# zdebruine/RcppML

Measured on AMD Instinct MI355X. Metric: ALS updates/sec (cols solved/s), k=64 sparse NMF, higher is better.
Workload: dtype f32; 1 GPU; configs[1]: simulateNMF 20000x100000 (x1 GPUs, column shards) 1%-dense CSC, k=64, MSE, coordinate-descent NNLS (cd_maxit=100, cd_tol=1e-8), L1 row normalisation, loss every iteration; rows=20000, cols_per_gpu=100000, nnz_per_gpu=20054852, k=64, solver=cd, cd_variant=auto, parallelism=column-shard x1

## Files before the change

### include/rcppml_gpu.h

```cpp
#ifndef RCPPML_GPU_H
#define RCPPML_GPU_H

#include <stddef.h>
#include <stdint.h>

#ifdef __cplusplus
extern "C" {
#endif

#define RCPPML_GPU_API __attribute__((visibility("default")))


RCPPML_GPU_API void rcppml_gpu_detect(int* num_gpus, double* total_mem_mb, double* free_mem_mb,
                                      int* max_gpus, int* out_status);

#define RCPPML_NMF_UNIFIED_ARGS                                                                    \
    const int* col_ptr, const int* row_idx, const double* values, int* m, int* n, int* nnz, int* k, \
        double* W, double* H, double* d, int* max_iter, double* tol, double* L1_H, double* L1_W,   \
        double* L2_H, double* L2_W, double* L21_H, double* L21_W, double* ortho_H, double* ortho_W, \
        double* ub_H, double* ub_W, int* cd_maxit, int* verbose, int* seed, int* loss_every,       \
        int* patience, int* nonneg_W, int* nonneg_H, int* loss_type, double* huber_delta,          \
        int* irls_max_iter, double* irls_tol, int* norm_type, int* projective, int* symmetric,     \
        int* solver_mode, const int* graph_W_p, const int* graph_W_i, const double* graph_W_x,     \
        int* graph_W_dim, int* graph_W_nnz, double* graph_W_lambda, const int* graph_H_p,          \
// ... 186 lines not shown
RCPPML_GPU_API void rcppml_gpu_consensus_double(const double* W_stack, int* m, int* k, int* reps, int* method, int* knn,
        double* out_consensus, int* out_labels, int* out_status);
RCPPML_GPU_API void rcppml_gpu_hclust_average_double(const double* dist, int* m, int* k_cut, int* out_merge, double* out_height,
        int* out_clusters, double* out_cophenetic, int* out_status);

RCPPML_GPU_API void rcppml_gpu_compute_target_double(const double* H, const int* labels, int* k, int* n, int* n_classes, int* whiten,
        double* out_target, double* out_shift, int* out_counts, int* out_status);
RCPPML_GPU_API void rcppml_gpu_refine_correct_double(const double* H, const int* labels, int* k, int* n, int* n_classes, int* whiten,
        double* lambda, int* nonneg, double* out_H_corr, double* out_target, int* out_status);
RCPPML_GPU_API void rcppml_gpu_refine_wfit_double(const int* col_ptr, const int* row_idx, const double* values, int* nnz,
        const double* dense, int* m, int* n, int* k, const double* d, const double* H_corr, int* nonneg, double* out_W,
        int* out_status);
RCPPML_GPU_API void rcppml_gpu_refine_double(const int* col_ptr, const int* row_idx, const double* values, int* nnz,
        const double* dense, int* m, int* n, int* k, const double* W_T, const double* d, const double* H, const int* labels,
        int* n_classes, double* lambda, int* cycles, int* nonneg, int* whiten, double* out_W, double* out_d, double* out_H,
        double* out_H_corr, int* out_status);

RCPPML_GPU_API void rcppml_gpu_nmf_zi_double(const int* col_ptr, const int* row_idx, const double* values, int* m, int* n, int* nnz,
        int* k, double* W, double* H, double* d, int* max_iter, double* tol, double* L1_H, double* L1_W, double* L2_H, double* L2_W,
        double* ub_H, double* ub_W, int* cd_maxit, double* cd_tol, int* verbose, int* patience, int* nonneg_W, int* nonneg_H,
        int* loss_type, int* irls_max_iter, double* irls_tol, int* norm_type, int* dispersion_mode, double* gp_theta_init,
        double* gp_theta_max, double* gp_theta_min, double* nb_size_init, double* nb_size_max, double* nb_size_min, int* sort_model,
        int* zi_mode, int* zi_em_iters, double* loss_history, double* out_theta, int* out_theta_len, double* out_pi, int* out_pi_len,
        int* out_iter, int* out_converged, double* out_loss, double* out_tol, int* out_status);
RCPPML_GPU_API void rcppml_gpu_zi_em_double(const int* col_ptr, const int* row_idx, const double* values, int* nnz, int* m, int* n,
        int* k, const double* W_T, const double* d, const double* H, double* disp, int* loss_type, int* zi_mode, int* zi_em_iters,
        double* theta_min, double* pi, double* out_imputed, int* out_status);

RCPPML_GPU_API const char* rcppml_gpu_last_error(void);

typedef struct rcppml_hip_ctx rcppml_hip_ctx;

enum { RCPPML_F32 = 0, RCPPML_F64 = 1 };
enum { RCPPML_CD_AUTO = 0 ,
       RCPPML_CD_LANE = 1 ,
       RCPPML_CD_WAVE = 2 ,
       RCPPML_CD_GROUP = 5 ,
       RCPPML_CD_MFMA16 = 7 ,
       RCPPML_CD_MFMA = 6 ,
       RCPPML_CD_LMF = 8  };

RCPPML_GPU_API int rcppml_hip_ctx_create(rcppml_hip_ctx** out, int device, void* stream);
RCPPML_GPU_API void rcppml_hip_ctx_destroy(rcppml_hip_ctx* ctx);
RCPPML_GPU_API int rcppml_hip_ctx_sync(rcppml_hip_ctx* ctx);
RCPPML_GPU_API int rcppml_hip_ctx_stats(rcppml_hip_ctx* ctx, int reset, unsigned long long* out4);
RCPPML_GPU_API int rcppml_hip_ctx_irls_stats(rcppml_hip_ctx* ctx, int reset, unsigned long long* out2);
RCPPML_GPU_API int rcppml_hip_ctx_irls_sweep_stats(rcppml_hip_ctx* ctx, int reset, unsigned long long* out1);
RCPPML_GPU_API int rcppml_hip_ctx_cd_step_stats(rcppml_hip_ctx* ctx, int reset, unsigned long long* out2);
enum { RCPPML_OPT_CD_COUNT_NOOP = 1 ,
       RCPPML_OPT_CD_LMF_LANE_GROUPS = 2 ,
       RCPPML_OPT_CD_LMF_WAVES_PER_SIMD = 3 ,
       RCPPML_OPT_CD_NO_LMF = 4 ,
       RCPPML_OPT_IRLS_COLUMNS_PER_WAVE = 5,
       RCPPML_OPT_SMALL_GIVE_UP = 6  };
RCPPML_GPU_API int rcppml_hip_ctx_set_option(rcppml_hip_ctx* ctx, int option, int value);

RCPPML_GPU_API int rcppml_hip_transpose_csc(rcppml_hip_ctx* ctx, int dtype, int rows, int cols, const int* col_ptr,
                                            const int* row_idx, const void* values, int* t_col_ptr, int* t_row_idx,
                                            void* t_values);
RCPPML_GPU_API int rcppml_hip_transpose_csc_sort(rcppml_hip_ctx* ctx, int rows, int cols, int64_t nnz, const int* col_ptr,
                                                 const int* row_idx, int* t_col_ptr, int* sorted_pos);
RCPPML_GPU_API int rcppml_hip_transpose_csc_gather(rcppml_hip_ctx* ctx, int dtype, int cols, int64_t nnz, const int* col_ptr,
                                                   const int* sorted_pos, const void* values, int* t_row_idx, void* t_values);
RCPPML_GPU_API int rcppml_hip_cast(rcppml_hip_ctx* ctx, int dtype_src, const void* src, int dtype_dst, void* dst, int64_t n);

RCPPML_GPU_API int rcppml_hip_gram(rcppml_hip_ctx* ctx, int dtype, const void* F, int k, int64_t r,
                                   double eps, double l2, void* G);

RCPPML_GPU_API int rcppml_hip_rhs(rcppml_hip_ctx* ctx, int dtype, const int* col_ptr,
                                  const int* row_idx, const void* values, int64_t ncols,
                                  const void* F, int k, void* B);

typedef struct rcppml_rhs_plan rcppml_rhs_plan;
RCPPML_GPU_API int rcppml_hip_rhs_plan_create(rcppml_hip_ctx* ctx, int dtype, const int* col_ptr, const int* row_idx,
                                              const void* values, int64_t ncols, int64_t nrows, int k, int partitions,
                                              int slots, rcppml_rhs_plan** out_plan);
RCPPML_GPU_API int rcppml_hip_rhs_plan_kind(const rcppml_rhs_plan* plan);
RCPPML_GPU_API int rcppml_hip_rhs_plan_create_indices(rcppml_hip_ctx* ctx, int dtype, const int* col_ptr, const int* row_idx, int64_t ncols,
                                                      int64_t nrows, int k, int partitions, int slots, rcppml_rhs_plan** out_plan);
RCPPML_GPU_API int rcppml_hip_rhs_plan_set_values(rcppml_hip_ctx* ctx, rcppml_rhs_plan* plan, const void* values);
RCPPML_GPU_API void rcppml_hip_rhs_plan_destroy(rcppml_rhs_plan* plan);
RCPPML_GPU_API int rcppml_hip_rhs_plan_info(const rcppml_rhs_plan* plan, double* out11);
RCPPML_GPU_API int rcppml_hip_rhs_planned(rcppml_hip_ctx* ctx, const rcppml_rhs_plan* plan, const void* F, void* B);

RCPPML_GPU_API int rcppml_hip_solve_cd(rcppml_hip_ctx* ctx, int dtype, const void* G, const void* B,
                                       void* X, int k, int64_t ncols, double l1_pre, int warm,
                                       int zero_init, double l1_cd, double l2_cd, int nonneg,
                                       int maxit, double tol, double ub_cd, double ub_post,
                                       int variant, int* sweeps_out, const int* col_order);

RCPPML_GPU_API int rcppml_hip_order_columns(rcppml_hip_ctx* ctx, const int* sweeps, int64_t ncols, int* order);

RCPPML_GPU_API int rcppml_hip_solve_chol(rcppml_hip_ctx* ctx, int dtype, const void* G,
                                         const void* B, void* X, int k, int64_t ncols,
                                         double l1_pre, int nonneg, double ub_post);

RCPPML_GPU_API int rcppml_hip_row_norms(rcppml_hip_ctx* ctx, int dtype, const void* X, int k,
                                        int64_t ncols, int norm_type, void* out);
RCPPML_GPU_API int rcppml_hip_apply_scaling(rcppml_hip_ctx* ctx, int dtype, void* X, int k,
                                            int64_t ncols, int norm_type, const void* sums, void* d);

RCPPML_GPU_API int rcppml_hip_scale_order(rcppml_hip_ctx* ctx, int dtype, void* X, int k, int64_t ncols, int norm_type,
                                          void* sums, void* d, const int* sweeps, int* order);

RCPPML_GPU_API int rcppml_hip_sumsq(rcppml_hip_ctx* ctx, int dtype, const void* x, int64_t len,
                                    double* out);

// ... 119 lines not shown
```

### rcppml_amd/_abi.py

```python
import ctypes as C
import os

import numpy as np

_HERE = os.path.dirname(os.path.abspath(__file__))
LIB_PATH = os.environ.get("RCPPML_GPU_LIB_PATH") or os.path.join(_HERE, "lib", "RcppML_gpu.so")
_lib = None

F32, F64 = 0, 1
CD_AUTO, CD_LANE, CD_WAVE, CD_GROUP, CD_MFMA, CD_MFMA16, CD_LMF = 0, 1, 2, 5, 6, 7, 8
OPT_CD_COUNT_NOOP, OPT_CD_LMF_LANE_GROUPS, OPT_CD_LMF_WAVES_PER_SIMD, OPT_CD_NO_LMF, OPT_IRLS_COLUMNS_PER_WAVE, OPT_SMALL_GIVE_UP = 1, 2, 3, 4, 5, 6

EXPORTED_SYMBOLS = [
    "rcppml_gpu_detect", "rcppml_gpu_nmf_unified_float", "rcppml_gpu_nmf_unified_double", "rcppml_gpu_nmf_ex",
    "rcppml_gpu_nmf_cv_unified_float", "rcppml_gpu_nmf_cv_unified_double", "rcppml_gpu_nmf_cv_ex", "rcppml_gpu_nmf_cv_irls_ex", "rcppml_gpu_nmf_cv_masked_ex", "rcppml_hip_ctx_set_cv_mask", "rcppml_gpu_nmf_zerocopy_double",
    "rcppml_gpu_nnls_double", "rcppml_gpu_evaluate_mse_double", "rcppml_gpu_nmf_profile_double", "rcppml_gpu_last_error",
    "rcppml_hip_ctx_create", "rcppml_hip_ctx_destroy", "rcppml_hip_ctx_sync", "rcppml_hip_ctx_stats", "rcppml_hip_ctx_irls_stats", "rcppml_hip_ctx_irls_sweep_stats", "rcppml_hip_ctx_cd_step_stats", "rcppml_hip_ctx_set_option", "rcppml_hip_transpose_csc", "rcppml_hip_transpose_csc_sort", "rcppml_hip_transpose_csc_gather", "rcppml_hip_cast", "rcppml_hip_gram", "rcppml_hip_rhs",
    "rcppml_hip_solve_cd", "rcppml_hip_order_columns", "rcppml_hip_solve_chol", "rcppml_hip_row_norms", "rcppml_hip_apply_scaling",
    "rcppml_hip_sumsq", "rcppml_hip_loss_mse", "rcppml_hip_solve_masked", "rcppml_hip_loss_nonzeros", "rcppml_hip_loss_masked",
    "rcppml_hip_solve_irls_nb", "rcppml_hip_nb_size_update", "rcppml_hip_nb_size_update_loss", "rcppml_hip_nb_loss", "rcppml_hip_solve_irls", "rcppml_hip_rhs_plan_kind", "rcppml_hip_irls_loss", "rcppml_hip_apply_l21", "rcppml_hip_angular_posthoc", "rcppml_hip_solve_cv", "rcppml_hip_cv_test_error", "rcppml_hip_solve_cv_irls", "rcppml_hip_cv_irls_loss", "rcppml_hip_cv_gp_theta_update", "rcppml_hip_mul_rows", "rcppml_hip_apply_graph_reg", "rcppml_hip_dispersion_update", "rcppml_hip_vec_global", "rcppml_hip_spz_info", "rcppml_hip_spz_decode",
    "rcppml_sp_read_gpu", "rcppml_sp_free_gpu", "rcppml_hip_rhs_dense", "rcppml_gpu_nmf_dense_unified_float",
    "rcppml_gpu_nmf_dense_unified_double",
    "rcppml_hip_rhs_plan_create", "rcppml_hip_rhs_plan_create_indices", "rcppml_hip_rhs_plan_set_values", "rcppml_hip_rhs_plan_destroy", "rcppml_hip_rhs_plan_info", "rcppml_hip_rhs_planned",
    "rcppml_gpu_nmf_target", "rcppml_hip_axpy", "rcppml_hip_add_diag", "rcppml_hip_clip_upper",
    "rcppml_hip_scale_order", "rcppml_hip_gram_loss_mse", "rcppml_hip_tail_scale_gram", "rcppml_hip_tail_scale_gram_loss",
    "rcppml_hip_als_small_eligible", "rcppml_hip_als_small_fit",
    "rcppml_gpu_bipartition_double", "rcppml_gpu_dclust_double", "rcppml_gpu_bipartition_ex", "rcppml_gpu_dclust_ex",
    "rcppml_gpu_svd_pca_double", "rcppml_gpu_svd_pca_float", "rcppml_gpu_svd_pca_dense_double", "rcppml_gpu_svd_pca_dense_float",
    "rcppml_gpu_assess", "rcppml_gpu_assess_ex", "rcppml_gpu_knn_float", "rcppml_gpu_assess_plan",
    "rcppml_gpu_score_test_double", "rcppml_gpu_zero_inflation_double", "rcppml_gpu_dispersion_double",
    "rcppml_gpu_consensus_double", "rcppml_gpu_hclust_average_double",
    "rcppml_gpu_compute_target_double", "rcppml_gpu_refine_correct_double", "rcppml_gpu_refine_wfit_double", "rcppml_gpu_refine_double",
    "rcppml_gpu_nmf_zi_double", "rcppml_gpu_zi_em_double",
]


class BackendError(RuntimeError):
    pass


class RhsPlan:

    def __init__(self, handle):
        self._h = handle

    def info(self):
        out = (C.c_double * 11)()
        lib().rcppml_hip_rhs_plan_info(self._h, out)
        keys = ("partitions", "waves", "rounds", "slots", "workgroups_per_partition", "tiles", "slot_count", "spilled_nnz",
                "fill", "stream_bytes", "tiled_columns")
        d = {k: (float(out[i]) if k == "fill" else int(out[i])) for i, k in enumerate(keys)}
        d["kind"] = {1: "window", 0: "slab"}.get(int(lib().rcppml_hip_rhs_plan_kind(self._h)), "?")
        d["slot_rate"] = float(out[3])
        return d

    def close(self):
        if self._h is not None and self._h.value:
            lib().rcppml_hip_rhs_plan_destroy(self._h)
            self._h = None

    def __del__(self):
        try:
            self.close()
        except Exception:
# ... 1082 lines not shown
```

### rcppml_amd/csrc/common.hip.h

```cpp
#pragma once
#include <hip/hip_runtime.h>

#include <cstdint>
#include <cstdio>
#include <cstdlib>
#include <cstring>
#include <mutex>
#include <stdexcept>
#include <string>
#include <type_traits>
#include <vector>

#include "../../include/rcppml_gpu.h"

inline std::string& rcppml_err() {
    static thread_local std::string e;
    return e;
}

#define HIPCHK(expr)                                                                             \
    do {                                                                                         \
        hipError_t _e = (expr);                                                                  \
        if (_e != hipSuccess)                                                                    \
            throw std::runtime_error(std::string(#expr) + " failed: " + hipGetErrorString(_e) +  \
                                     " (" __FILE__ ":" + std::to_string(__LINE__) + ")");        \
    } while (0)

#define RCPPML_CATCH_RET                                      \
    catch (const std::exception& e) {                         \
        rcppml_err() = e.what();                              \
        return 1;                                             \
    }                                                         \
    catch (...) {                                             \
        rcppml_err() = "unknown error";                       \
        return 1;                                             \
    }

#ifdef RCPPML_EXPERIMENTS
inline bool exp_flag(const char* name, const char* value) { const char* e = getenv(name); return e && !strcmp(e, value); }
inline const char* exp_env(const char* name) { return getenv(name); }
#else
inline bool exp_flag(const char*, const char*) { return false; }
inline const char* exp_env(const char*) { return nullptr; }
#endif

struct rcppml_hip_ctx;
enum { WS_GRAM = 0, WS_GPAD, WS_CHOL, WS_RED, WS_RED2, WS_ORDER, WS_IRLS, WS_MFMA, WS_FEAT, WS_GRAPH, WS_COUNT };

struct DynSmemOnce {
    size_t set_bytes[32] = {};
    std::mutex mu;
    void ensure(const void* fn, size_t smem, int device) {
        const int d = device & 31;
        std::lock_guard<std::mutex> lk(mu);
        if (smem > 48 * 1024 && smem > set_bytes[d]) {
            const hipError_t e = hipFuncSetAttribute(fn, hipFuncAttributeMaxDynamicSharedMemorySize, (int)smem);
            if (e != hipSuccess) {
                (void)hipGetLastError();
                throw std::runtime_error("this kernel needs " + std::to_string(smem) + " bytes of LDS per workgroup, more than device " +
                                         std::to_string(device) + " grants (" + hipGetErrorString(e) +
                                         "): the configuration (rank above 64?) needs gfx950's 160 KiB of LDS per CU");
            }
            set_bytes[d] = smem;
        }
    }
};

struct rcppml_hip_ctx {
    int device = 0;
    hipStream_t stream = nullptr;
    int num_cu = 256;
    const int* cv_mask_p[2] = {nullptr, nullptr};
    const int* cv_mask_i[2] = {nullptr, nullptr};
    struct Buf { void* ptr = nullptr; size_t bytes = 0; };
    Buf bufs[WS_COUNT];
    unsigned long long* stats = nullptr;
    int opt_cd_count = 0, opt_lmf_lg = 0, opt_lmf_wps = 0, opt_cd_no_lmf = 0, opt_irls_cpw = 0, opt_small_give_up = 0;
    char* arena = nullptr;
    size_t arena_cap = 0, arena_off = 0;
    void* arena_take(size_t bytes) {
        const size_t a = (arena_off + 255) & ~(size_t)255;
        if (!arena || a + bytes > arena_cap) return nullptr;
        arena_off = a + bytes;
        return arena + a;
    }
    void* scratch(int slot, size_t bytes) {
        Buf& b = bufs[slot];
        if (bytes > b.bytes) {
            if (b.ptr) HIPCHK(hipFree(b.ptr));
            b.ptr = nullptr; b.bytes = 0;
            size_t want = bytes < 4096 ? 4096 : bytes;
            HIPCHK(hipMalloc(&b.ptr, want));
            b.bytes = want;
        }
        return b.ptr;
    }
};

struct DevTmp {
    void* p = nullptr;
    bool owned = false;
    DevTmp(rcppml_hip_ctx* c, size_t bytes) {
        if (bytes < 16) bytes = 16;
        p = c ? c->arena_take(bytes) : nullptr;
        if (!p) { HIPCHK(hipMalloc(&p, bytes)); owned = true; }
    }
    ~DevTmp() { if (p && owned) (void)hipFree(p); }
    DevTmp(const DevTmp&) = delete;
    DevTmp& operator=(const DevTmp&) = delete;
};
```

### rcppml_amd/csrc/kernels_cd_mfma64.hip.h

```cpp
#pragma once
#include "kernels.hip.h"

namespace rk {

template <class T> struct Vec4T;
template <> struct Vec4T<float> { typedef float4 type; };
template <> struct Vec4T<double> { typedef double4 type; };
template <int P> __device__ __forceinline__ unsigned bcast_row32(unsigned a) {
    if constexpr (P == 2) {
        return __builtin_amdgcn_permlane16_swap(a, a, false, false)[0];
    } else {
        const auto tu = __builtin_amdgcn_permlane16_swap(a, a, false, false);
        if constexpr (P == 0) {
            return __builtin_amdgcn_permlane32_swap(tu[0], tu[0], false, false)[0];
        } else {
            return __builtin_amdgcn_permlane32_swap(tu[1], tu[1], false, false)[0];
        }
    }
}
template <int P> __device__ __forceinline__ float bcast_row(float a) {
    return __uint_as_float(bcast_row32<P>(__float_as_uint(a)));
}
template <int P> __device__ __forceinline__ double bcast_row(double a) {
    const unsigned long long u = __double_as_longlong(a);
    const unsigned lo = bcast_row32<P>((unsigned)u), hi = bcast_row32<P>((unsigned)(u >> 32));
    return __longlong_as_double(((unsigned long long)hi << 32) | lo);
}

template <class T> struct CdStepOut64 { T a, nx; };
__device__ __forceinline__ float tmax(float a, float b) { return __builtin_fmaxf(a, b); }
__device__ __forceinline__ double tmax(double a, double b) { return __builtin_fmax(a, b); }

template <bool SIMPLE, class T>
__device__ __forceinline__ CdStepOut64<T> cd_step64(T b, T xo, T gd, T ginv, bool active, T l1_cd, T l2_cd, T lo, T hi) {
    CdStepOut64<T> o;
    if constexpr (SIMPLE) {
        const T diff = cd_quotient(b, gd, ginv);
        o.a = tmax(diff, -xo);
        o.nx = tmax(xo + diff, T(0));
    } else {
        T diff = cd_quotient(b, gd, ginv);
        diff -= l1_cd;
        diff = tfma(l2_cd, xo, diff);
        const T nv = xo + diff;
        const bool neg = nv < lo, up = nv > hi;
        T nx = neg ? lo : (up ? hi : nv);
        T a = neg ? lo - xo : (up ? hi - xo : diff);
        const bool on = active && (ginv > T(0));
        o.a = on ? a : T(0);
        o.nx = on ? nx : xo;
    }
    return o;
}

__device__ __forceinline__ f64x4 mfma16(double a, double b, f64x4 c) { return __builtin_amdgcn_mfma_f64_16x16x4f64(a, b, c, 0, 0, 0); }
typedef float f32x4 __attribute__((ext_vector_type(4)));
__device__ __forceinline__ f32x4 mfma16(float a, float b, f32x4 c) { return __builtin_amdgcn_mfma_f32_16x16x4f32(a, b, c, 0, 0, 0); }
template <class T> struct Acc4T;
template <> struct Acc4T<float> { typedef f32x4 type; };
template <> struct Acc4T<double> { typedef f64x4 type; };
__device__ __forceinline__ float fast_recip(float den) { return __builtin_amdgcn_rcpf(den); }
__device__ __forceinline__ double fast_recip(double den) {
    const double rc = __builtin_amdgcn_rcp(den);
    return __builtin_fma(__builtin_fma(-den, rc, 1.0), rc, rc);
}

template <class T, int NT, bool SIMPLE>
__global__ __launch_bounds__(256) __attribute__((amdgpu_waves_per_eu(NT <= 2 ? 4 : (NT <= 4 ? 2 : 1), 8)))
void cd_mfma64_kernel(const T* __restrict__ G , const T* __restrict__ B,
                      T* __restrict__ X, int k, int64_t ncols, T l1_pre, int warm, int zero_init, T l1_cd,
                      T l2_cd, int nonneg, int maxit, T tol, T ub_cd, T ub_post,
                      int* __restrict__ sweeps, const int* __restrict__ order, unsigned long long* __restrict__ stats) {
    typedef typename Vec4T<T>::type Tab4;
    typedef typename Acc4T<T>::type Acc4;
    constexpr int KP = 16 * NT;
    extern __shared__ __attribute__((aligned(16))) char smem_raw[];
    T* Gs = reinterpret_cast<T*>(smem_raw);
    Tab4* tab_s = reinterpret_cast<Tab4*>(Gs + KP * KP);
    [[maybe_unused]] T* gd_s = Gs + KP * KP + 4 * KP;
    {
        constexpr bool PERM = sizeof(T) == 4;
        auto gp = [&](int col, int row) { return (row < k && col < k) ? G[(int64_t)col * k + row] : (row == col ? T(1) : T(0)); };
        for (int e = threadIdx.x; e < KP * KP; e += blockDim.x) {
            const int qt = e >> 6, kk = (e >> 4) & 3, ps = e & 15;
            const int q = qt / NT, t = qt % NT;
            const int rl = PERM ? (ps >> 2) + 4 * (ps & 3) : ps;
            Gs[e] = -gp(4 * q + kk, 16 * t + rl);
        }
        for (int c = threadIdx.x; c < KP; c += blockDim.x) {
            const int gg = c & 3, qb = c & ~3;
            Tab4 v;
            const T gd = gp(c, c);
            v.x = gd > T(0) ? T(1) / gd : T(0);
            v.y = gg > 0 ? gp(qb + 0, c) : T(0);
            v.z = gg > 1 ? gp(qb + 1, c) : T(0);
            v.w = gg > 2 ? gp(qb + 2, c) : T(0);
            tab_s[c] = v;
            if constexpr (sizeof(T) == 8) gd_s[c] = gd > T(0) ? gd : T(0);
        }
    }
    __syncthreads();
    const int wave = threadIdx.x >> 6, lane = threadIdx.x & 63;
    const int g = lane >> 4, cl = lane & 15;
    const int64_t base = ((int64_t)blockIdx.x * (blockDim.x >> 6) + wave) * 16;
    if (base >= ncols) return;
    const int64_t slot = base + cl;
    const bool inb = slot < ncols;
    const int64_t j = (inb && order) ? order[slot] : slot;
    Acc4 acc[NT];
    T xr[NT][4];
    {
        const T* bj = B + j * (int64_t)k;
        const T* xj = X + j * (int64_t)k;
#pragma unroll
        for (int t = 0; t < NT; ++t)
#pragma unroll
            for (int v = 0; v < 4; ++v) {
                const int row = 16 * t + 4 * v + g;
                const bool ok = inb && row < k;
                T bv = ok ? bj[row] : T(0);
                if (ok && l1_pre != T(0)) bv -= l1_pre;
                acc[t][v] = bv;
                xr[t][v] = (ok && !zero_init) ? xj[row] : T(0);
            }
    }
    if (warm) {
#pragma unroll
        for (int t = 0; t < NT; ++t)
#pragma unroll
            for (int v = 0; v < 4; ++v) {
                const int q = 4 * t + v;
#pragma unroll
                for (int t2 = 0; t2 < NT; ++t2) {
                    const T av = Gs[((q * NT + t2) << 6) + lane];
                    acc[t2] = mfma16(av, xr[t][v], acc[t2]);
                }
            }
    }
    const T lo = nonneg ? T(0) : -INFINITY;
    const T hi = ub_cd > T(0) ? ub_cd : INFINITY;
    const bool check = tol > T(0);
    const T inv_k = T(1) / static_cast<T>(k);
    bool active = inb;
    int nsweep = 0;
    Tab4 tb_c = tab_s[g];
    [[maybe_unused]] T gd_c = T(0);
    if constexpr (sizeof(T) == 8) gd_c = gd_s[g];
    T av_c[NT];
#pragma unroll
    for (int t2 = 0; t2 < NT; ++t2) av_c[t2] = Gs[(t2 << 6) + lane];
    for (int it = 0; it < maxit; ++it) {
        if (!__any(active)) break;
        T tsum = T(0);
        nsweep += active ? 1 : 0;
#pragma unroll
        for (int t = 0; t < NT; ++t)
#pragma unroll
            for (int v = 0; v < 4; ++v) {
                constexpr int NQ = KP / 4;
                const int qn = (4 * t + v + 1) % NQ;
                const int tn = (v == 3 ? t + 1 : t) % NT;
                const Tab4 tb_n = tab_s[4 * qn + g];
                [[maybe_unused]] T gd_n = T(0);
                if constexpr (sizeof(T) == 8) gd_n = gd_s[4 * qn + g];
                T av_n[NT];
#pragma unroll
                for (int t2 = 0; t2 < NT; ++t2) av_n[t2] = Gs[((qn * NT + t2) << 6) + lane];
                const T b0 = acc[t][v];
                const T xo = xr[t][v];
                const T ginv = SIMPLE ? (active ? tb_c.x : T(0)) : tb_c.x;
                const CdStepOut64<T> s0 = cd_step64<SIMPLE, T>(b0, xo, gd_c, ginv, active, l1_cd, l2_cd, lo, hi);
                const T b1 = tfma(-tb_c.y, bcast_row<0>(s0.a), b0);
                const CdStepOut64<T> s1 = cd_step64<SIMPLE, T>(b1, xo, gd_c, ginv, active, l1_cd, l2_cd, lo, hi);
                const T b2 = tfma(-tb_c.z, bcast_row<1>(s1.a), b1);
                const CdStepOut64<T> s2 = cd_step64<SIMPLE, T>(b2, xo, gd_c, ginv, active, l1_cd, l2_cd, lo, hi);
                const T b3 = tfma(-tb_c.w, bcast_row<2>(s2.a), b2);
                const CdStepOut64<T> s3 = cd_step64<SIMPLE, T>(b3, xo, gd_c, ginv, active, l1_cd, l2_cd, lo, hi);
                xr[t][v] = s3.nx;
                tsum = tfma(tabs(s3.a), fast_recip(tabs(s3.nx) + T(1e-15)), tsum);
#pragma unroll
                for (int s = 0; s < NT; ++s) {
                    const int t2 = (tn + s) % NT;
                    acc[t2] = mfma16(av_c[t2], s3.a, acc[t2]);
                }
                tb_c = tb_n;
                gd_c = gd_n;
#pragma unroll
                for (int t2 = 0; t2 < NT; ++t2) av_c[t2] = av_n[t2];
                __builtin_amdgcn_sched_barrier(0);
            }
        T tot = tsum + __shfl_xor(tsum, 16, 64);
        tot += __shfl_xor(tot, 32, 64);
        active = active && !(check && tot * inv_k < tol);
    }
    if (inb) {
        T* xj = X + j * (int64_t)k;
#pragma unroll
        for (int t = 0; t < NT; ++t)
#pragma unroll
            for (int v = 0; v < 4; ++v) {
                const int row = 16 * t + 4 * v + g;
                if (row < k) {
                    T val = xr[t][v];
                    if (ub_post > T(0)) val = val < ub_post ? val : ub_post;
                    xj[row] = val;
                }
            }
        if (sweeps && g == 0) sweeps[j] = nsweep;
    }
    cd_stats_add(stats, (inb && g == 0) ? nsweep : 0, (inb && g == 0) ? 1 : 0);
}

}
```

### rcppml_amd/csrc/ops_gram.hip

```cpp
#include "common.hip.h"
#include "kernels.hip.h"
#include "gram_launch.hip.h"

using namespace rk;
extern "C" int rcppml_hip_ctx_create(rcppml_hip_ctx** out, int device, void* stream) {
    try {
        int ndev = 0;
        HIPCHK(hipGetDeviceCount(&ndev));
        if (ndev <= 0) throw std::runtime_error("no HIP device visible");
        if (device < 0 || device >= ndev) throw std::runtime_error("device index out of range");
        HIPCHK(hipSetDevice(device));
        rcppml_hip_ctx* c = new rcppml_hip_ctx();
        c->device = device;
        c->stream = static_cast<hipStream_t>(stream);
        hipDeviceProp_t prop;
        HIPCHK(hipGetDeviceProperties(&prop, device));
        c->num_cu = prop.multiProcessorCount;
        HIPCHK(hipMalloc(&c->stats, 12 * sizeof(unsigned long long)));
        HIPCHK(hipMemset(c->stats, 0, 12 * sizeof(unsigned long long)));
        *out = c;
        return 0;
    }
    RCPPML_CATCH_RET
}
extern "C" void rcppml_hip_ctx_destroy(rcppml_hip_ctx* c) {
    if (!c) return;
    for (auto& b : c->bufs)
        if (b.ptr) (void)hipFree(b.ptr);
    if (c->stats) (void)hipFree(c->stats);
    delete c;
}
extern "C" int rcppml_hip_ctx_sync(rcppml_hip_ctx* c) {
    try { HIPCHK(hipStreamSynchronize(c->stream)); return 0; }
    RCPPML_CATCH_RET
}
extern "C" int rcppml_hip_ctx_set_option(rcppml_hip_ctx* c, int option, int value) {
    if (!c) return 1;
    switch (option) {
        case RCPPML_OPT_CD_COUNT_NOOP: c->opt_cd_count = value; return 0;
        case RCPPML_OPT_CD_LMF_LANE_GROUPS: c->opt_lmf_lg = value; return 0;
        case RCPPML_OPT_CD_LMF_WAVES_PER_SIMD: c->opt_lmf_wps = value; return 0;
        case RCPPML_OPT_CD_NO_LMF: c->opt_cd_no_lmf = value; return 0;
        case RCPPML_OPT_IRLS_COLUMNS_PER_WAVE: c->opt_irls_cpw = value; return 0;
        case RCPPML_OPT_SMALL_GIVE_UP: c->opt_small_give_up = value; return 0;
        default: rcppml_err() = "unknown option"; return 1;
    }
}
extern "C" int rcppml_hip_ctx_stats(rcppml_hip_ctx* c, int reset, unsigned long long* out4) {
    try {
        HIPCHK(hipStreamSynchronize(c->stream));
        if (out4) HIPCHK(hipMemcpy(out4, c->stats, 4 * sizeof(unsigned long long), hipMemcpyDeviceToHost));
        if (reset) HIPCHK(hipMemset(c->stats, 0, 4 * sizeof(unsigned long long)));
        return 0;
    }
    RCPPML_CATCH_RET
}
extern "C" int rcppml_hip_ctx_cd_step_stats(rcppml_hip_ctx* c, int reset, unsigned long long* out2) {
    try {
        HIPCHK(hipSetDevice(c->device));
        HIPCHK(hipStreamSynchronize(c->stream));
        if (out2) HIPCHK(hipMemcpy(out2, c->stats + 6, 2 * sizeof(unsigned long long), hipMemcpyDeviceToHost));
        if (reset) HIPCHK(hipMemset(c->stats + 6, 0, 2 * sizeof(unsigned long long)));
        return 0;
    }
    RCPPML_CATCH_RET
}
extern "C" int rcppml_hip_ctx_irls_stats(rcppml_hip_ctx* c, int reset, unsigned long long* out2) {
    try {
        HIPCHK(hipStreamSynchronize(c->stream));
        if (out2) HIPCHK(hipMemcpy(out2, c->stats + 4, 2 * sizeof(unsigned long long), hipMemcpyDeviceToHost));
        if (reset) HIPCHK(hipMemset(c->stats + 4, 0, 2 * sizeof(unsigned long long)));
        return 0;
    }
    RCPPML_CATCH_RET
}

extern "C" int rcppml_hip_ctx_irls_sweep_stats(rcppml_hip_ctx* c, int reset, unsigned long long* out1) {
    try {
        HIPCHK(hipStreamSynchronize(c->stream));
        if (out1) HIPCHK(hipMemcpy(out1, c->stats + 8, sizeof(unsigned long long), hipMemcpyDeviceToHost));
        if (reset) HIPCHK(hipMemset(c->stats + 8, 0, sizeof(unsigned long long)));
        return 0;
    }
    RCPPML_CATCH_RET
}

template <class T>
static void gram_impl(rcppml_hip_ctx* c, const T* F, int k, int64_t r, T eps, T l2, T* G) {
    int nblk = 0, KP = 0;
    const T* partial = gram_partials<T>(c, F, k, r, &nblk, &KP);
    hipLaunchKernelGGL(gram_finalize<T>, dim3((KP * KP + 7) / 8), dim3(256), 0, c->stream, partial, nblk, KP, k, eps, l2, G);
    HIPCHK(hipGetLastError());
}
extern "C" int rcppml_hip_gram(rcppml_hip_ctx* c, int dtype, const void* F, int k, int64_t r, double eps,
                               double l2, void* G) {
    try {
        HIPCHK(hipSetDevice(c->device));
// ... 8 lines not shown
```

### rcppml_amd/csrc/solve_cd_impl.hip.h

```cpp
#pragma once
#include <cmath>
#include "solve_common.hip.h"
#include "kernels_cd_mfma.hip.h"
#include "kernels_cd_mfma64.hip.h"
template <class T, int KP>
static void cd_lane_launch(rcppml_hip_ctx* c, const T* Gp, const T* invd, const T* B, T* X, int k,
                           int64_t ncols, T l1_pre, int warm, int zero_init, T l1_cd, T l2_cd, int nonneg,
                           int maxit, T tol, T ub_cd, T ub_post, int* sweeps, const int* order) {
    constexpr bool EXACT = std::is_same<T, double>::value;
    const int64_t nblk = (ncols + 63) / 64;
    hipLaunchKernelGGL((cd_lane_kernel<T, KP, EXACT>), dim3((unsigned)nblk), dim3(64), 0, c->stream, Gp, invd,
                       B, X, k, ncols, l1_pre, warm, zero_init, l1_cd, l2_cd, nonneg, maxit, tol, ub_cd, ub_post, sweeps, order);
    HIPCHK(hipGetLastError());
}
template <class T, int KP, bool GLDS = true>
static void cd_wave_launch(rcppml_hip_ctx* c, const T* Gp, const T* invd, const T* B, T* X, int k,
                           int64_t ncols, T l1_pre, int warm, int zero_init, T l1_cd, T l2_cd, int nonneg,
                           int maxit, T tol, T ub_cd, T ub_post, int* sweeps, const int* order) {
    constexpr bool EXACT = std::is_same<T, double>::value;
    const size_t smem = GLDS ? (size_t)KP * KP * sizeof(T) : 0;
    auto kern = cd_wave_kernel<T, KP, EXACT, GLDS>;
    static DynSmemOnce once;
    once.ensure(reinterpret_cast<const void*>(kern), smem, c->device);
    int per_cu = (int)((160 * 1024) / (smem + 256));
// ... 18 lines not shown
    auto kern = cd_group_kernel<T, KP, LPC, EXACT>;
    static DynSmemOnce once;
    once.ensure(reinterpret_cast<const void*>(kern), smem, c->device);
    const int64_t per_block = (int64_t)4 * (64 / LPC);
    const int64_t nblk = (ncols + per_block - 1) / per_block;
    hipLaunchKernelGGL(kern, dim3((unsigned)nblk), dim3(256), smem, c->stream, Gp, invd, B, X, k, ncols, l1_pre, warm,
                       zero_init, l1_cd, l2_cd, nonneg, maxit, tol, ub_cd, ub_post, sweeps, order, c->stats);
    HIPCHK(hipGetLastError());
}

template <int RT, int CT>
static void cd_mfma_launch(rcppml_hip_ctx* c, const float* G, const float* , const float* B, float* X, int k,
                           int64_t ncols, float l1_pre, int warm, int zero_init, float l1_cd, float l2_cd, int nonneg,
                           int maxit, float tol, float ub_cd, float ub_post, int* sweeps, const int* order) {
    size_t smem = cd_mfma_lds_bytes(RT);
    const int64_t per_block = 4 * 32 * CT;
    const int64_t nblk = (ncols + per_block - 1) / per_block;
    const bool simple = nonneg && ub_cd <= 0.f && l1_cd == 0.f && l2_cd == 0.f;
    {
        const double per_cu = (double)nblk / (double)(c->num_cu > 0 ? c->num_cu : 256);
        int cap = 0;
        if (per_cu > 1.0 && per_cu < 4.0 && per_cu - std::floor(per_cu) < 0.5) cap = (int)std::floor(per_cu);
        if (const char* e = exp_env("RCPPML_GPU_CD_CAP")) cap = atoi(e);
        if (cap > 0) {
            const size_t lds_cu = 160 * 1024;
            const size_t want = lds_cu / (size_t)(cap + 1) + 1024;
            if (want > smem && want <= lds_cu / (size_t)cap) smem = want;
        }
    }
    static DynSmemOnce once_simple, once_general;
    if (simple) once_simple.ensure(reinterpret_cast<const void*>(&cd_mfma_kernel<RT, CT, true>), smem, c->device);
    else once_general.ensure(reinterpret_cast<const void*>(&cd_mfma_kernel<RT, CT, false>), smem, c->device);
    if (simple)
        hipLaunchKernelGGL((cd_mfma_kernel<RT, CT, true>), dim3((unsigned)nblk), dim3(256), smem, c->stream, G, B, X,
                           k, ncols, l1_pre, warm, zero_init, l1_cd, l2_cd, nonneg, maxit, tol, ub_cd, ub_post, sweeps, order, c->stats);
    else
        hipLaunchKernelGGL((cd_mfma_kernel<RT, CT, false>), dim3((unsigned)nblk), dim3(256), smem, c->stream, G, B, X,
                           k, ncols, l1_pre, warm, zero_init, l1_cd, l2_cd, nonneg, maxit, tol, ub_cd, ub_post, sweeps, order, c->stats);
    HIPCHK(hipGetLastError());
}


void rcppml_cd_lmf_dispatch(rcppml_hip_ctx* c, const float* G, const float* B, float* X, int k, int64_t ncols, float l1_pre,
                            int warm, int zero_init, int maxit, float tol, float ub_post, int* sweeps, const int* order);

template <class T, int NT>
static void cd_mfma64_launch(rcppml_hip_ctx* c, const T* G, const T* , const T* B, T* X, int k,
                             int64_t ncols, T l1_pre, int warm, int zero_init, T l1_cd, T l2_cd, int nonneg,
                             int maxit, T tol, T ub_cd, T ub_post, int* sweeps, const int* order) {
    constexpr int KP = 16 * NT;
    const size_t smem = ((size_t)KP * KP + 4 * KP + (sizeof(T) == 8 ? KP : 0)) * sizeof(T);
    const int64_t nblk = (ncols + 63) / 64;
    const bool simple = nonneg && ub_cd <= T(0) && l1_cd == T(0) && l2_cd == T(0);
    static DynSmemOnce once_simple, once_general;
    if (simple) once_simple.ensure(reinterpret_cast<const void*>(&cd_mfma64_kernel<T, NT, true>), smem, c->device);
    else once_general.ensure(reinterpret_cast<const void*>(&cd_mfma64_kernel<T, NT, false>), smem, c->device);
    if (simple)
        hipLaunchKernelGGL((cd_mfma64_kernel<T, NT, true>), dim3((unsigned)nblk), dim3(256), smem, c->stream, G, B, X, k,
                           ncols, l1_pre, warm, zero_init, l1_cd, l2_cd, nonneg, maxit, tol, ub_cd, ub_post, sweeps, order, c->stats);
    else
        hipLaunchKernelGGL((cd_mfma64_kernel<T, NT, false>), dim3((unsigned)nblk), dim3(256), smem, c->stream, G, B, X, k,
                           ncols, l1_pre, warm, zero_init, l1_cd, l2_cd, nonneg, maxit, tol, ub_cd, ub_post, sweeps, order, c->stats);
    HIPCHK(hipGetLastError());
}

template <class T>
static int pick_lpc(int KP) {
    const int ev = 16 / (int)sizeof(T);
    const char* e = exp_env("RCPPML_GPU_CD_LPC");
    int lpc = e ? atoi(e) : (std::is_same<T, float>::value ? KP / 32 : KP / 16);
    if (lpc < 1) lpc = 1;
    if (lpc > 4) lpc = 4;
    while (lpc < 4 && KP / lpc > 32) lpc *= 2;
    while (lpc > 1 && (KP / lpc) % ev != 0) lpc /= 2;
    return lpc;
}

template <class T>
static void solve_cd_impl(rcppml_hip_ctx* c, const T* G, const T* B, T* X, int k, int64_t ncols, T l1_pre,
                          int warm, int zero_init, T l1_cd, T l2_cd, int nonneg, int maxit, T tol, T ub_cd,
                          T ub_post, int variant, int* sweeps, const int* order) {
    if (ncols <= 0) return;
    if (k < 1 || k > 256) throw std::runtime_error("solve_cd: k must be in [1,256]");
    if (k > 128) {
        T *Gp, *invd;
        pad_impl<T>(c, G, k, 256, &Gp, &invd);
        cd_wave_launch<T, 256, false>(c, Gp, invd, B, X, k, ncols, l1_pre, warm, zero_init, l1_cd, l2_cd, nonneg, maxit, tol, ub_cd,
                                      ub_post, sweeps, order);
        return;
    }
    int KP = solve_kp(k);
    const bool lmf_ok = std::is_same<T, float>::value && k <= 64 && nonneg && ub_cd <= T(0) && l1_cd == T(0) && l2_cd == T(0) && maxit >= 1;
    if (variant == RCPPML_CD_LMF && !lmf_ok) variant = RCPPML_CD_AUTO;
    if (variant == RCPPML_CD_AUTO && lmf_ok && k <= 32 && ncols >= (int64_t)256 * c->num_cu && !c->opt_cd_no_lmf &&
        !exp_env("RCPPML_GPU_CD_VARIANT"))
        variant = RCPPML_CD_LMF;
    if (variant == RCPPML_CD_LMF) {
        if constexpr (std::is_same<T, float>::value)
            rcppml_cd_lmf_dispatch(c, G, B, X, k, ncols, l1_pre, warm, zero_init, maxit, tol, ub_post, sweeps, order);
        return;
    }
    if (variant == RCPPML_CD_AUTO && k <= 64 && nonneg && ub_cd <= T(0) && l1_cd == T(0) && l2_cd == T(0) && maxit >= 1 &&
        ncols <= (int64_t)6 * (c->num_cu > 0 ? c->num_cu : 256) && !exp_env("RCPPML_GPU_CD_VARIANT")) {
        const unsigned nblk = (unsigned)((ncols + 3) / 4);
        if (k <= 16)
            hipLaunchKernelGGL((cd_wave_static_kernel<T, 16>), dim3(nblk), dim3(256), 0, c->stream, G, B, X, k, ncols, l1_pre, warm, zero_init,
                               maxit, tol, ub_post, sweeps, c->stats);
        else if (k <= 32)
            hipLaunchKernelGGL((cd_wave_static_kernel<T, 32>), dim3(nblk), dim3(256), 0, c->stream, G, B, X, k, ncols, l1_pre, warm, zero_init,
                               maxit, tol, ub_post, sweeps, c->stats);
// ... 82 lines not shown
```

Before: 106.6 million cols/s.

## Keep Gram image in registers for simple fp32 CD MFMA64 solver

Adds a register-resident variant of the 64-wide MFMA coordinate-descent kernel for fp32 simple nonneg problems with k<=64. It preloads the Gram tiles and step tables into registers instead of reading LDS on every update. It stores X negated so the nonneg clamp becomes a single min, and spreads the MFMA updates between the dependent scalar steps to hide latency. Converged columns zero their accumulators. The cost is much higher register pressure and possibly lower occupancy; an option falls back to the LDS path.

```diff
diff --git a/include/rcppml_gpu.h b/include/rcppml_gpu.h
--- a/include/rcppml_gpu.h
+++ b/include/rcppml_gpu.h
@@ -262,7 +262,8 @@
        RCPPML_OPT_CD_LMF_WAVES_PER_SIMD = 3 ,
        RCPPML_OPT_CD_NO_LMF = 4 ,
        RCPPML_OPT_IRLS_COLUMNS_PER_WAVE = 5,
-       RCPPML_OPT_SMALL_GIVE_UP = 6  };
+       RCPPML_OPT_SMALL_GIVE_UP = 6 ,
+       RCPPML_OPT_CD16_LDS = 7  };
 RCPPML_GPU_API int rcppml_hip_ctx_set_option(rcppml_hip_ctx* ctx, int option, int value);
 
 RCPPML_GPU_API int rcppml_hip_transpose_csc(rcppml_hip_ctx* ctx, int dtype, int rows, int cols, const int* col_ptr,
diff --git a/rcppml_amd/_abi.py b/rcppml_amd/_abi.py
--- a/rcppml_amd/_abi.py
+++ b/rcppml_amd/_abi.py
@@ -10,6 +10,7 @@
 F32, F64 = 0, 1
 CD_AUTO, CD_LANE, CD_WAVE, CD_GROUP, CD_MFMA, CD_MFMA16, CD_LMF = 0, 1, 2, 5, 6, 7, 8
 OPT_CD_COUNT_NOOP, OPT_CD_LMF_LANE_GROUPS, OPT_CD_LMF_WAVES_PER_SIMD, OPT_CD_NO_LMF, OPT_IRLS_COLUMNS_PER_WAVE, OPT_SMALL_GIVE_UP = 1, 2, 3, 4, 5, 6
+OPT_CD16_LDS = 7
 
 EXPORTED_SYMBOLS = [
     "rcppml_gpu_detect", "rcppml_gpu_nmf_unified_float", "rcppml_gpu_nmf_unified_double", "rcppml_gpu_nmf_ex",
diff --git a/rcppml_amd/csrc/common.hip.h b/rcppml_amd/csrc/common.hip.h
--- a/rcppml_amd/csrc/common.hip.h
+++ b/rcppml_amd/csrc/common.hip.h
@@ -75,7 +75,7 @@
     struct Buf { void* ptr = nullptr; size_t bytes = 0; };
     Buf bufs[WS_COUNT];
     unsigned long long* stats = nullptr;
-    int opt_cd_count = 0, opt_lmf_lg = 0, opt_lmf_wps = 0, opt_cd_no_lmf = 0, opt_irls_cpw = 0, opt_small_give_up = 0;
+    int opt_cd_count = 0, opt_lmf_lg = 0, opt_lmf_wps = 0, opt_cd_no_lmf = 0, opt_irls_cpw = 0, opt_small_give_up = 0, opt_cd16_lds = 0;
     char* arena = nullptr;
     size_t arena_cap = 0, arena_off = 0;
     void* arena_take(size_t bytes) {
diff --git a/rcppml_amd/csrc/kernels_cd_mfma64.hip.h b/rcppml_amd/csrc/kernels_cd_mfma64.hip.h
--- a/rcppml_amd/csrc/kernels_cd_mfma64.hip.h
+++ b/rcppml_amd/csrc/kernels_cd_mfma64.hip.h
@@ -1,5 +1,6 @@
 #pragma once
 #include "kernels.hip.h"
+#include "kernels_cd_mfma.hip.h"
 
 namespace rk {
 
@@ -17,6 +18,10 @@
             return __builtin_amdgcn_permlane32_swap(tu[1], tu[1], false, false)[0];
         }
     }
+}
+__device__ __forceinline__ float bcast_row2_inplace(float a) {
+    asm volatile("s_nop 1\n\tv_permlane16_swap_b32 %0, %0" : "+v"(a));
+    return a;
 }
 template <int P> __device__ __forceinline__ float bcast_row(float a) {
     return __uint_as_float(bcast_row32<P>(__float_as_uint(a)));
@@ -65,7 +70,7 @@
     return __builtin_fma(__builtin_fma(-den, rc, 1.0), rc, rc);
 }
 
-template <class T, int NT, bool SIMPLE>
+template <class T, int NT, bool SIMPLE, bool REGS = false>
 __global__ __launch_bounds__(256) __attribute__((amdgpu_waves_per_eu(NT <= 2 ? 4 : (NT <= 4 ? 2 : 1), 8)))
 void cd_mfma64_kernel(const T* __restrict__ G , const T* __restrict__ B,
                       T* __restrict__ X, int k, int64_t ncols, T l1_pre, int warm, int zero_init, T l1_cd,
@@ -74,6 +79,8 @@
     typedef typename Vec4T<T>::type Tab4;
     typedef typename Acc4T<T>::type Acc4;
     constexpr int KP = 16 * NT;
+    static_assert(!REGS || (sizeof(T) == 4 && SIMPLE && NT <= 4), "register-resident image: fp32, SIMPLE, k <= 64");
+    constexpr T XSIGN = REGS ? T(-1) : T(1);
     extern __shared__ __attribute__((aligned(16))) char smem_raw[];
     T* Gs = reinterpret_cast<T*>(smem_raw);
     Tab4* tab_s = reinterpret_cast<Tab4*>(Gs + KP * KP);
@@ -109,6 +116,16 @@
     const int64_t j = (inb && order) ? order[slot] : slot;
     Acc4 acc[NT];
     T xr[NT][4];
+    [[maybe_unused]] Tab4 tab_r[REGS ? 4 * NT : 1];
+    [[maybe_unused]] T av_r[REGS ? 4 * NT : 1][NT];
+    if constexpr (REGS) {
+#pragma unroll
+        for (int q = 0; q < 4 * NT; ++q) {
+            tab_r[q] = tab_s[4 * q + g];
+#pragma unroll
+            for (int t2 = 0; t2 < NT; ++t2) av_r[q][t2] = Gs[((q * NT + t2) << 6) + lane];
+        }
+    }
     {
         const T* bj = B + j * (int64_t)k;
         const T* xj = X + j * (int64_t)k;
@@ -121,7 +138,7 @@
                 T bv = ok ? bj[row] : T(0);
                 if (ok && l1_pre != T(0)) bv -= l1_pre;
                 acc[t][v] = bv;
-                xr[t][v] = (ok && !zero_init) ? xj[row] : T(0);
+                xr[t][v] = (ok && !zero_init) ? XSIGN * xj[row] : T(0);
             }
     }
     if (warm) {
@@ -132,8 +149,10 @@
                 const int q = 4 * t + v;
 #pragma unroll
                 for (int t2 = 0; t2 < NT; ++t2) {
-                    const T av = Gs[((q * NT + t2) << 6) + lane];
-                    acc[t2] = mfma16(av, xr[t][v], acc[t2]);
+                    T av;
+                    if constexpr (REGS) av = av_r[q][t2];
+                    else av = Gs[((q * NT + t2) << 6) + lane];
+                    acc[t2] = mfma16(av, XSIGN * xr[t][v], acc[t2]);
                 }
             }
     }
@@ -143,55 +162,118 @@
     const T inv_k = T(1) / static_cast<T>(k);
     bool active = inb;
     int nsweep = 0;
-    Tab4 tb_c = tab_s[g];
-    [[maybe_unused]] T gd_c = T(0);
-    if constexpr (sizeof(T) == 8) gd_c = gd_s[g];
-    T av_c[NT];
-#pragma unroll
-    for (int t2 = 0; t2 < NT; ++t2) av_c[t2] = Gs[(t2 << 6) + lane];
-    for (int it = 0; it < maxit; ++it) {
-        if (!__any(active)) break;
-        T tsum = T(0);
-        nsweep += active ? 1 : 0;
-#pragma unroll
-        for (int t = 0; t < NT; ++t)
-#pragma unroll
-            for (int v = 0; v < 4; ++v) {
-                constexpr int NQ = KP / 4;
-                const int qn = (4 * t + v + 1) % NQ;
-                const int tn = (v == 3 ? t + 1 : t) % NT;
-                const Tab4 tb_n = tab_s[4 * qn + g];
-                [[maybe_unused]] T gd_n = T(0);
-                if constexpr (sizeof(T) == 8) gd_n = gd_s[4 * qn + g];
-                T av_n[NT];
-#pragma unroll
-                for (int t2 = 0; t2 < NT; ++t2) av_n[t2] = Gs[((qn * NT + t2) << 6) + lane];
-                const T b0 = acc[t][v];
-                const T xo = xr[t][v];
-                const T ginv = SIMPLE ? (active ? tb_c.x : T(0)) : tb_c.x;
-                const CdStepOut64<T> s0 = cd_step64<SIMPLE, T>(b0, xo, gd_c, ginv, active, l1_cd, l2_cd, lo, hi);
-                const T b1 = tfma(-tb_c.y, bcast_row<0>(s0.a), b0);
-                const CdStepOut64<T> s1 = cd_step64<SIMPLE, T>(b1, xo, gd_c, ginv, active, l1_cd, l2_cd, lo, hi);
-                const T b2 = tfma(-tb_c.z, bcast_row<1>(s1.a), b1);
-                const CdStepOut64<T> s2 = cd_step64<SIMPLE, T>(b2, xo, gd_c, ginv, active, l1_cd, l2_cd, lo, hi);
-                const T b3 = tfma(-tb_c.w, bcast_row<2>(s2.a), b2);
-                const CdStepOut64<T> s3 = cd_step64<SIMPLE, T>(b3, xo, gd_c, ginv, active, l1_cd, l2_cd, lo, hi);
-                xr[t][v] = s3.nx;
-                tsum = tfma(tabs(s3.a), fast_recip(tabs(s3.nx) + T(1e-15)), tsum);
-#pragma unroll
-                for (int s = 0; s < NT; ++s) {
-                    const int t2 = (tn + s) % NT;
-                    acc[t2] = mfma16(av_c[t2], s3.a, acc[t2]);
-                }
-                tb_c = tb_n;
-                gd_c = gd_n;
-#pragma unroll
-                for (int t2 = 0; t2 < NT; ++t2) av_c[t2] = av_n[t2];
-                __builtin_amdgcn_sched_barrier(0);
-            }
-        T tot = tsum + __shfl_xor(tsum, 16, 64);
-        tot += __shfl_xor(tot, 32, 64);
-        active = active && !(check && tot * inv_k < tol);
+    if constexpr (REGS) {
+        for (int it = 0; it < maxit; ++it) {
+            if (!__any(active)) break;
+            T tsum = T(0);
+            nsweep += active ? 1 : 0;
+            T a_prev = T(0);
+#pragma unroll
+            for (int t = 0; t < NT; ++t)
+#pragma unroll
+                for (int v = 0; v < 4; ++v) {
+                    constexpr int NQ = KP / 4;
+                    const int q = 4 * t + v;
+                    const int tn = (v == 3 ? t + 1 : t) % NT;
+                    auto due = [&](int s) {
+                        if (q > 0 && s < NT) {
+                            const int t2 = (t + s) % NT;
+                            __builtin_amdgcn_sched_barrier(0);
+                            acc[t2] = mfma16(av_r[(q + NQ - 1) % NQ][t2], a_prev, acc[t2]);
+                            __builtin_amdgcn_sched_barrier(0);
+                        }
+                    };
+                    const Tab4 tb = tab_r[q];
+                    const T xs = xr[t][v];
+                    const T b0 = acc[t][v];
+                    const T a0 = cd_max_nc(b0 * tb.x, xs, hi);
+                    due(1);
+                    const T b1 = tfma(-tb.y, bcast_row<0>(a0), b0);
+                    const T a1 = cd_max_nc(b1 * tb.x, xs, hi);
+                    due(2);
+                    const T b2 = tfma(-tb.z, bcast_row<1>(a1), b1);
+                    const T a2 = cd_max_nc(b2 * tb.x, xs, hi);
+                    due(3);
+                    const T b3 = tfma(-tb.w, bcast_row2_inplace(a2), b2);
+                    const T d3 = b3 * tb.x;
+                    const T a3 = cd_max_nc(d3, xs, hi);
+                    acc[tn] = mfma16(av_r[q][tn], a3, acc[tn]);
+                    __builtin_amdgcn_sched_barrier(0);
+                    const T nxs = __builtin_fminf(tfma(-tb.x, b3, xs), T(0));
+                    xr[t][v] = nxs;
+                    tsum = tfma(tabs(a3), fast_recip(tabs(nxs) + T(1e-15)), tsum);
+                    a_prev = a3;
+                    if (q == NQ - 1) {
+#pragma unroll
+                        for (int s = 1; s < NT; ++s) {
+                            const int t2 = (tn + s) % NT;
+                            acc[t2] = mfma16(av_r[q][t2], a3, acc[t2]);
+                        }
+                    }
+                    __builtin_amdgcn_sched_barrier(0);
+                }
+            T tot = tsum + __shfl_xor(tsum, 16, 64);
+            tot += __shfl_xor(tot, 32, 64);
+            const bool now = active && !(check && tot * inv_k < tol);
+            if (__any(active && !now)) {
+#pragma unroll
+                for (int t = 0; t < NT; ++t)
+#pragma unroll
+                    for (int v = 0; v < 4; ++v) acc[t][v] = now ? acc[t][v] : T(0);
+            }
+            active = now;
+        }
+    } else {
+        Tab4 tb_c = tab_s[g];
+        [[maybe_unused]] T gd_c = T(0);
+        if constexpr (sizeof(T) == 8) gd_c = gd_s[g];
+        T av_c[NT];
+#pragma unroll
+        for (int t2 = 0; t2 < NT; ++t2) av_c[t2] = Gs[(t2 << 6) + lane];
+        for (int it = 0; it < maxit; ++it) {
+            if (!__any(active)) break;
+            T tsum = T(0);
+            nsweep += active ? 1 : 0;
+#pragma unroll
+            for (int t = 0; t < NT; ++t)
+#pragma unroll
+                for (int v = 0; v < 4; ++v) {
+                    constexpr int NQ = KP / 4;
+                    const int qn = (4 * t + v + 1) % NQ;
+                    const int tn = (v == 3 ? t + 1 : t) % NT;
+                    const Tab4 tb_n = tab_s[4 * qn + g];
+                    [[maybe_unused]] T gd_n = T(0);
+                    if constexpr (sizeof(T) == 8) gd_n = gd_s[4 * qn + g];
+                    T av_n[NT];
+#pragma unroll
+                    for (int t2 = 0; t2 < NT; ++t2) av_n[t2] = Gs[((qn * NT + t2) << 6) + lane];
+                    const T b0 = acc[t][v];
+                    const T xo = xr[t][v];
+                    const T ginv = SIMPLE ? (active ? tb_c.x : T(0)) : tb_c.x;
+                    const CdStepOut64<T> s0 = cd_step64<SIMPLE, T>(b0, xo, gd_c, ginv, active, l1_cd, l2_cd, lo, hi);
+                    const T b1 = tfma(-tb_c.y, bcast_row<0>(s0.a), b0);
+                    const CdStepOut64<T> s1 = cd_step64<SIMPLE, T>(b1, xo, gd_c, ginv, active, l1_cd, l2_cd, lo, hi);
+                    const T b2 = tfma(-tb_c.z, bcast_row<1>(s1.a), b1);
+                    const CdStepOut64<T> s2 = cd_step64<SIMPLE, T>(b2, xo, gd_c, ginv, active, l1_cd, l2_cd, lo, hi);
+                    const T b3 = tfma(-tb_c.w, bcast_row<2>(s2.a), b2);
+                    const CdStepOut64<T> s3 = cd_step64<SIMPLE, T>(b3, xo, gd_c, ginv, active, l1_cd, l2_cd, lo, hi);
+                    xr[t][v] = s3.nx;
+                    tsum = tfma(tabs(s3.a), fast_recip(tabs(s3.nx) + T(1e-15)), tsum);
+#pragma unroll
+                    for (int s = 0; s < NT; ++s) {
+                        const int t2 = (tn + s) % NT;
+                        acc[t2] = mfma16(av_c[t2], s3.a, acc[t2]);
+                    }
+                    tb_c = tb_n;
+                    gd_c = gd_n;
+#pragma unroll
+                    for (int t2 = 0; t2 < NT; ++t2) av_c[t2] = av_n[t2];
+                    __builtin_amdgcn_sched_barrier(0);
+                }
+            T tot = tsum + __shfl_xor(tsum, 16, 64);
+            tot += __shfl_xor(tot, 32, 64);
+            active = active && !(check && tot * inv_k < tol);
+        }
     }
     if (inb) {
         T* xj = X + j * (int64_t)k;
@@ -201,7 +283,7 @@
             for (int v = 0; v < 4; ++v) {
                 const int row = 16 * t + 4 * v + g;
                 if (row < k) {
-                    T val = xr[t][v];
+                    T val = REGS ? T(0) - xr[t][v] : xr[t][v];
                     if (ub_post > T(0)) val = val < ub_post ? val : ub_post;
                     xj[row] = val;
                 }
diff --git a/rcppml_amd/csrc/ops_gram.hip b/rcppml_amd/csrc/ops_gram.hip
--- a/rcppml_amd/csrc/ops_gram.hip
+++ b/rcppml_amd/csrc/ops_gram.hip
@@ -43,6 +43,7 @@
         case RCPPML_OPT_CD_NO_LMF: c->opt_cd_no_lmf = value; return 0;
         case RCPPML_OPT_IRLS_COLUMNS_PER_WAVE: c->opt_irls_cpw = value; return 0;
         case RCPPML_OPT_SMALL_GIVE_UP: c->opt_small_give_up = value; return 0;
+        case RCPPML_OPT_CD16_LDS: c->opt_cd16_lds = value; return 0;
         default: rcppml_err() = "unknown option"; return 1;
     }
 }
diff --git a/rcppml_amd/csrc/solve_cd_impl.hip.h b/rcppml_amd/csrc/solve_cd_impl.hip.h
--- a/rcppml_amd/csrc/solve_cd_impl.hip.h
+++ b/rcppml_amd/csrc/solve_cd_impl.hip.h
@@ -94,10 +94,16 @@
     const size_t smem = ((size_t)KP * KP + 4 * KP + (sizeof(T) == 8 ? KP : 0)) * sizeof(T);
     const int64_t nblk = (ncols + 63) / 64;
     const bool simple = nonneg && ub_cd <= T(0) && l1_cd == T(0) && l2_cd == T(0);
-    static DynSmemOnce once_simple, once_general;
-    if (simple) once_simple.ensure(reinterpret_cast<const void*>(&cd_mfma64_kernel<T, NT, true>), smem, c->device);
+    constexpr bool CAN_REGS = std::is_same<T, float>::value && NT <= 4;
+    const bool regs = CAN_REGS && simple && !c->opt_cd16_lds;
+    static DynSmemOnce once_regs, once_simple, once_general;
+    if (regs) once_regs.ensure(reinterpret_cast<const void*>(&cd_mfma64_kernel<T, NT, true, CAN_REGS>), smem, c->device);
+    else if (simple) once_simple.ensure(reinterpret_cast<const void*>(&cd_mfma64_kernel<T, NT, true>), smem, c->device);
     else once_general.ensure(reinterpret_cast<const void*>(&cd_mfma64_kernel<T, NT, false>), smem, c->device);
-    if (simple)
+    if (regs)
+        hipLaunchKernelGGL((cd_mfma64_kernel<T, NT, true, CAN_REGS>), dim3((unsigned)nblk), dim3(256), smem, c->stream, G, B, X, k,
+                           ncols, l1_pre, warm, zero_init, l1_cd, l2_cd, nonneg, maxit, tol, ub_cd, ub_post, sweeps, order, c->stats);
+    else if (simple)
         hipLaunchKernelGGL((cd_mfma64_kernel<T, NT, true>), dim3((unsigned)nblk), dim3(256), smem, c->stream, G, B, X, k,
                            ncols, l1_pre, warm, zero_init, l1_cd, l2_cd, nonneg, maxit, tol, ub_cd, ub_post, sweeps, order, c->stats);
     else
```

After: 104.2 million cols/s. 0.978x the previous value.
